# yzqin/s4g-release

Hardware: AMD Instinct MI355X
Metric: scenes/sec (25.6k-pt clouds) end-to-end grasp inference (higher is better)
Workload: dtype f32 (f16x2 split)

## Files before the change

s4g_release_amd/csrc/mlp_gemm.hip:

```cpp
#include <stdlib.h>

#include "mlp_common.h"

#include <type_traits>

#ifndef S4G_CHAIN_ABLATE
#define S4G_CHAIN_ABLATE 0
#endif

namespace s4g {


constexpr int GM_BM = 128;
constexpr int GM_BN = 128;
constexpr int GM_BK = 32;
constexpr int GM_LDS = 36;
constexpr int GM_THREADS = 256;

enum { LOAD_PLAIN = 0, LOAD_GATHER = 1, LOAD_INTERP = 2, LOAD_GATHER_MLP1 = 3, LOAD_GATHER_ADD = 4,
       LOAD_INTERP_ADD = 5, LOAD_CHANNEL_FIRST = 6,
       LOAD_REL_MLP1 = 64,
       LOAD_ADD_MFMA0 = 65 };
enum { EPI_STORE = 0, EPI_MAX = 1, EPI_CHANNEL_FIRST = 2, EPI_MAX_CF = 3 };

struct GemmParams {
  int P, Cin, Kpad, Cout, relu;
  const float* W;
  const float* bias;
  const float* A;
  int lda, a_coff, a_gcol;
  int aL;
  const int* gidx;
  const float* feat;
  const float* xyz;
  const float* ctr;
  int Cf, N, M, K;
  int nscenes;
  const float4* mlp1;
  const float4* rel4;
  const int* seg4;
  const int* seg_rows;
  float* out2;
  int ldc2, split_n;
  uint32_t* out_amax2;
  const int* nidx;
  const float* nw;
  const float* sparse;
  const float* dense;
  int C2, C1, N2, N1;
  float* out;
  int ldc, c_coff, c_gcol;
  int w_gstride, b_gstride;
  float* cf_ptr[4];
  int cf_start[5];
  int cf_sigmoid_from;
  int cf_N;
  int mtiles, ntiles;
  const uint16_t* W3;
  int Kpad16;
  int bf16_single;
  size_t w3_plane;
  const uint16_t* Wh2;
  const float* w_inv_scale;
  const float* a_amax;
  const float* a_amax2;
  float a_amax_floor;
  uint32_t* out_amax;
  int rps;
  const uint16_t* Wfrag;
  const float* lbias;
  const uint16_t* Wfrag2;
  const float* w_inv_scale2;
  const float* bias2;
  int Cout2, relu2;
  const uint16_t* Wfrag3;
  const float* w_inv_scale3;
  const float* bias3;
  int Cout3, relu3;
};

__device__ __forceinline__ float4 f4zero() { return make_float4(0.f, 0.f, 0.f, 0.f); }

__device__ __forceinline__ void gather_row_bm(int M, int K, int p0, int r, int& b, int& m) {
  const int MK = M * K;
  const int b0 = __builtin_amdgcn_readfirstlane(p0 / MK);
  int rem = p0 - b0 * MK + r;
  b = b0;
  while (rem >= MK) {
    rem -= MK;
    ++b;
  }
  m = (K & (K - 1)) == 0 ? rem >> (31 - __clz(K)) : rem / K;
}

template <int LOADER, int RPT = 4, int RS = 32>
struct ALoader {
  static __device__ __forceinline__ int srow(int t) { return LOADER == LOAD_CHANNEL_FIRST ? (t & 31) : (t >> 3); }
  static __device__ __forceinline__ int chunk(int t) { return LOADER == LOAD_CHANNEL_FIRST ? (t >> 5) : (t & 7); }
  const float* src0[RPT];
  bool ok[RPT];
  float rel[RPT][3];
  int i3[RPT][3];
  float w3[RPT][3];
  size_t drow[RPT];

  __device__ __forceinline__ void init(const GemmParams& p, int p0, int g, int t) {
    constexpr bool GATHERS = LOADER == LOAD_GATHER_MLP1 || LOADER == LOAD_GATHER_ADD || LOADER == LOAD_GATHER;
    int pp_[RPT], j_[RPT], b_[RPT], m_[RPT];
#pragma unroll
    for (int s = 0; s < RPT; ++s) {
      const int r = srow(t) + RS * s;
      const int pos = p0 + r;
      ok[s] = pos < p.P;
      pp_[s] = ok[s] ? pos : 0;
      j_[s] = b_[s] = m_[s] = 0;
      if constexpr (GATHERS) {
        if (!(LOADER == LOAD_GATHER_MLP1 && p.rel4)) {
          gather_row_bm(p.M, p.K, p0, ok[s] ? r : 0, b_[s], m_[s]);
          j_[s] = p.gidx[pp_[s]];
        }
      }
    }
#pragma unroll
    for (int s = 0; s < RPT; ++s) {
      const int pp = pp_[s], j = j_[s], b = b_[s], m = m_[s];
      if constexpr (LOADER == LOAD_PLAIN) {
        src0[s] = p.A + (size_t)pp * p.lda + p.a_coff + g * p.a_gcol;
      } else if constexpr (LOADER == LOAD_CHANNEL_FIRST) {
        const int b = pp / p.aL;
        src0[s] = p.A + (size_t)b * p.Cin * p.aL + (pp - b * p.aL);
      } else if constexpr (LOADER == LOAD_GATHER_MLP1) {
        if (p.rel4) {
          const float4 r4 = p.rel4[pp];
          rel[s][0] = r4.x;
          rel[s][1] = r4.y;
          rel[s][2] = r4.z;
          continue;
        }
        const float* x = p.xyz + (size_t)b * 3 * p.N;
        const float* c = p.ctr + (size_t)b * 3 * p.M;
        rel[s][0] = __fsub_rn(x[j], c[m]);
        rel[s][1] = __fsub_rn(x[p.N + j], c[p.M + m]);
        rel[s][2] = __fsub_rn(x[2 * p.N + j], c[2 * p.M + m]);
      } else if constexpr (LOADER == LOAD_GATHER_ADD) {
        src0[s] = p.feat + ((size_t)b * p.N + j) * p.Cf;
        const float* x = p.xyz + (size_t)b * 3 * p.N;
        const float* c = p.ctr + (size_t)b * 3 * p.M;
        rel[s][0] = __fsub_rn(x[j], c[m]);
        rel[s][1] = __fsub_rn(x[p.N + j], c[p.M + m]);
        rel[s][2] = __fsub_rn(x[2 * p.N + j], c[2 * p.M + m]);
      } else if constexpr (LOADER == LOAD_GATHER) {
        src0[s] = p.feat ? p.feat + ((size_t)b * p.N + j) * p.Cf : nullptr;
        if ((t & 7) == ((p.Cf & 31) >> 2)) {
          const float* x = p.xyz + (size_t)b * 3 * p.N;
          const float* c = p.ctr + (size_t)b * 3 * p.M;
          rel[s][0] = __fsub_rn(x[j], c[m]);
          rel[s][1] = __fsub_rn(x[p.N + j], c[p.M + m]);
          rel[s][2] = __fsub_rn(x[2 * p.N + j], c[2 * p.M + m]);
        }
      } else {
        const int bq = pp / p.N1;
#pragma unroll
        for (int k = 0; k < 3; ++k) {
          i3[s][k] = bq * p.N2 + p.nidx[(size_t)pp * 3 + k];
          w3[s][k] = p.nw[(size_t)pp * 3 + k];
        }
        drow[s] = (size_t)pp;
      }
    }
  }

  __device__ __forceinline__ float4 load(const GemmParams& p, int s, int k0, int t) const {
    if constexpr (LOADER == LOAD_GATHER_MLP1) {
      const bool live = ok[s] && k0 < p.Cin;
      const int kk = k0 < p.Cin ? k0 : 0;
      float4 r;
      float* rp = reinterpret_cast<float*>(&r);
#pragma unroll
      for (int e = 0; e < 4; ++e) {
        const float4 w = p.mlp1[kk + e];
        const float v = __fmaf_rn(w.z, rel[s][2], __fmaf_rn(w.y, rel[s][1], __fmaf_rn(w.x, rel[s][0], w.w)));
        rp[e] = live ? fmaxf(v, 0.f) : 0.f;
      }
      return r;
    }
    if constexpr (LOADER == LOAD_GATHER_ADD) {
      const bool live = ok[s] && k0 < p.Cin;
      const int kk = k0 < p.Cin ? k0 : 0;
      const float4 f = *reinterpret_cast<const float4*>(src0[s] + kk);
      const float fv[4] = {f.x, f.y, f.z, f.w};
      float4 r;
      float* rp = reinterpret_cast<float*>(&r);
#pragma unroll
      for (int e = 0; e < 4; ++e) {
        const float4 w = p.mlp1[kk + e];
        const float v = __fmaf_rn(w.z, rel[s][2], __fmaf_rn(w.y, rel[s][1], __fmaf_rn(w.x, rel[s][0], w.w)));
        rp[e] = live ? fmaxf(__fadd_rn(fv[e], v), 0.f) : 0.f;
// ... 986 lines not shown
    f32x16 z16;
#pragma unroll
    for (int r = 0; r < 16; ++r) z16[r] = 0.f;
#pragma unroll
    for (int rb = 0; rb < NRB; ++rb)
      asm volatile("s_nop 7" : "+v"(af0[rb][0].x), "+v"(af0[rb][0].y), "+v"(af0[rb][1].x), "+v"(af0[rb][1].y));
    __builtin_amdgcn_sched_barrier(0);
#pragma unroll
    for (int cb = 0; cb < 2; ++cb)
#pragma unroll
      for (int rb = 0; rb < NRB; ++rb) {
        acc[cb][rb] = chain_mfma<PL>(bf0[cb][1], af0[rb][0], z16);
        acc[cb][rb] = chain_mfma<PL>(bf0[cb][0], af0[rb][1], acc[cb][rb]);
        acc[cb][rb] = chain_mfma<PL>(bf0[cb][0], af0[rb][0], acc[cb][rb]);
      }
    if constexpr (ADD0) {
      float* Fs = smemf;
#pragma unroll
      for (int kt = 0; kt < NKT0; ++kt)
#pragma unroll
        for (int s = 0; s < RPT; ++s)
          *reinterpret_cast<float4*>(Fs + ((t >> 3) + RS * s) * fstr + kt * 32 + (t & 7) * 4) = fa[kt][s];
      __syncthreads();
#pragma unroll
      for (int nb = 0; nb < 2; ++nb)
#pragma unroll
        for (int j = 0; j < 4; ++j) {
          const float4 f4 = *reinterpret_cast<const float4*>(epi_s + nb * 32 + 8 * j + 4 * lh);
#pragma unroll
          for (int pb = 0; pb < NRB; ++pb) {
            const float4 fv = *reinterpret_cast<const float4*>(Fs + (wr * WROWS + pb * 32 + li) * fstr + wc * 64 + nb * 32 +
                                                               8 * j + 4 * lh);
            acc[nb][pb][4 * j] = __fmaf_rn(acc[nb][pb][4 * j], f4.x, fv.x);
            acc[nb][pb][4 * j + 1] = __fmaf_rn(acc[nb][pb][4 * j + 1], f4.y, fv.y);
            acc[nb][pb][4 * j + 2] = __fmaf_rn(acc[nb][pb][4 * j + 2], f4.z, fv.z);
            acc[nb][pb][4 * j + 3] = __fmaf_rn(acc[nb][pb][4 * j + 3], f4.w, fv.w);
          }
        }
      __syncthreads();
#pragma unroll
      for (int nb = 0; nb < 2; ++nb)
#pragma unroll
        for (int j = 0; j < 4; ++j)
#pragma unroll
          for (int pb = 0; pb < NRB; ++pb) {
            uint16_t* dst = Ah + (wr * WROWS + pb * 32 + li) * astr + wc * 64 + nb * 32 + 8 * j + 4 * lh;
            uint2 h, l;
            split_quad_h(fmaxf(acc[nb][pb][4 * j], 0.f), fmaxf(acc[nb][pb][4 * j + 1], 0.f),
                         fmaxf(acc[nb][pb][4 * j + 2], 0.f), fmaxf(acc[nb][pb][4 * j + 3], 0.f), sa, h.x, l.x, h.y, l.y);
            *reinterpret_cast<uint2*>(dst) = h;
            *reinterpret_cast<uint2*>(dst + aplane) = l;
          }
    } else {
#pragma unroll
      for (int nb = 0; nb < 2; ++nb)
#pragma unroll
        for (int j = 0; j < 4; ++j) {
          const float4 f4 = *reinterpret_cast<const float4*>(epi_s + nb * 32 + 8 * j + 4 * lh);
#pragma unroll
          for (int pb = 0; pb < NRB; ++pb) {
            uint16_t* dst = Ah + (wr * WROWS + pb * 32 + li) * astr + wc * 64 + nb * 32 + 8 * j + 4 * lh;
            uint2 h, l;
            split_quad_h2(fmaxf(acc[nb][pb][4 * j], 0.f), fmaxf(acc[nb][pb][4 * j + 1], 0.f),
                          fmaxf(acc[nb][pb][4 * j + 2], 0.f), fmaxf(acc[nb][pb][4 * j + 3], 0.f), f4.x, f4.y, f4.z, f4.w,
                          h.x, l.x, h.y, l.y);
            *reinterpret_cast<uint2*>(dst) = h;
            *reinterpret_cast<uint2*>(dst + aplane) = l;
          }
        }
    }
  } else {
    if (!(S4G_CHAIN_ABLATE & 16)) load_panel(0, std::integral_constant<int, (K / 32) / (NRB / 2)>{});
  }
  S4G_STAMP(2);
  __syncthreads();
  S4G_STAMP(3);

  auto zero_acc = [&]() {
#pragma unroll
    for (int i = 0; i < 2; ++i)
#pragma unroll
      for (int j = 0; j < NRB; ++j)
#pragma unroll
        for (int r = 0; r < 16; ++r) acc[i][j][r] = 0.f;
  };
  uint4 afn[NRB][PL];
  auto prime_a = [&]() {
#pragma unroll
    for (int rb = 0; rb < NRB; ++rb)
#pragma unroll
      for (int pl = 0; pl < PL; ++pl)
        afn[rb][pl] = *reinterpret_cast<const uint4*>(a_lane + pl * aplane + rb * 32 * astr);
  };

#define S4G_F2_STRIP(SWAPPED, ZFIRST, wcur, cbs_cur, wnext, cbs_next)                                                     \
  _Pragma("unroll") for (int ks = 0; ks < KS; ++ks) {                                                  \
    const int d = ks % GF_RING;                                                                        \
    const int ksn = ks + 1 == KS ? 0 : ks + 1;                                                         \
    uint4 af[NRB][PL], bf[2][PL];                                                                      \
    _Pragma("unroll") for (int rb = 0; rb < NRB; ++rb) _Pragma("unroll") for (int pl = 0; pl < PL; ++pl) { \
      af[rb][pl] = afn[rb][pl];                                                                        \
      if (!(S4G_CHAIN_ABLATE & 2))                                                                     \
        afn[rb][pl] = *reinterpret_cast<const uint4*>(a_lane + pl * aplane + rb * 32 * astr + ksn * 16); \
    }                                                                                                  \
    _Pragma("unroll") for (int cb = 0; cb < 2; ++cb) _Pragma("unroll") for (int pl = 0; pl < PL; ++pl)  \
      bf[cb][pl] = ring[d][cb][pl];                                                                    \
    {                                                                                                  \
      const int kr = ks + GF_RING;                                                                     \
      const WRef src = kr < KS ? (wcur) : (wnext);                                                     \
      const size_t cbs = kr < KS ? (cbs_cur) : (cbs_next);                                             \
      const int kk = kr < KS ? kr : kr - KS;                                                           \
      _Pragma("unroll") for (int cb = 0; cb < 2; ++cb) _Pragma("unroll") for (int pl = 0; pl < PL; ++pl) \
        if (!(S4G_CHAIN_ABLATE & 1))                                                                   \
          ring[d][cb][pl] = wref_load(src, wf_lane + pl * 1024, (uint32_t)(cb * cbs + (size_t)kk * PL * 1024)); \
    }                                                                                                  \
    if constexpr (PL == 2) {                                                                           \
      S4G_F2_TERM(SWAPPED, 0, 1, (ZFIRST) && ks == 0)                                                  \
      S4G_F2_TERM(SWAPPED, 1, 0, false)                                                                \
      S4G_F2_TERM(SWAPPED, 0, 0, false)                                                                \
    } else {                                                                                           \
      S4G_F2_TERM(SWAPPED, 0, 0, (ZFIRST) && ks == 0)                                                  \
    }                                                                                                  \
    _Pragma("unroll") for (int q = 0; q < 2 * PL; ++q) {                                               \
      __builtin_amdgcn_sched_group_barrier(0x008, 1, 0);                                               \
      __builtin_amdgcn_sched_group_barrier(0x100, 1, 0);                                               \
      __builtin_amdgcn_sched_group_barrier(0x008, 1, 0);                                               \
      __builtin_amdgcn_sched_group_barrier(0x020, 1, 0);                                               \
    }                                                                                                  \
    if constexpr (PL == 2) __builtin_amdgcn_sched_group_barrier(0x008, 4, 0);                          \
    if constexpr (PL == 1 && NRB == 4) {             \
      _Pragma("unroll") for (int q = 0; q < 2; ++q) {                                                  \
        __builtin_amdgcn_sched_group_barrier(0x100, 1, 0);                                             \
        __builtin_amdgcn_sched_group_barrier(0x008, 2, 0);                                             \
      }                                                                                                \
    }                                                                                                  \
    __builtin_amdgcn_sched_barrier(0);                                                                 \
  }
#define S4G_F2_TERM(SWAPPED, PA, PB, Z)                                                                \
  _Pragma("unroll") for (int cb = 0; cb < 2; ++cb) _Pragma("unroll") for (int rb = 0; rb < NRB; ++rb)  \
    if constexpr (SWAPPED)                                                                             \
      acc[cb][rb] = chain_mfma<PL>(bf[cb][PB], af[rb][PA], (Z) ? zero16 : acc[cb][rb]);                \
    else                                                                                               \
      acc[cb][rb] = chain_mfma<PL>(af[rb][PA], bf[cb][PB], (Z) ? zero16 : acc[cb][rb]);
  f32x16 zero16;
#pragma unroll
  for (int r = 0; r < 16; ++r) zero16[r] = 0.f;

  WRef wcur = w1;
  const float* __restrict__ scp = PL == 2 ? p.w_inv_scale + (size_t)g * p.b_gstride : nullptr;
  const float* __restrict__ bp = p.bias + (size_t)g * p.b_gstride;
  int relu_ph = p.relu;
  float inv_in = inv_sa, inv_sh = 1.f;
  const int npanel = tri ? 2 : 1;
  for (int ph = 0; ph < npanel; ++ph) {
  const WRef wnxt = ph + 1 < npanel ? wmid : (active0 ? w2 : wcur);
  prime_a();
  {
    const int n = wc * 64 + lane;
    epi_s[lane] = PL == 2 ? inv_in * scp[n] : 1.f;
    epi_s[64 + lane] = bp[n];
  }
  if (KC > 1 && ph == 0) {
    zero_acc();
    for (int kc = 0; kc < kchunks; ++kc) {
      if (kc > 0) {
        __syncthreads();
        load_panel(kc, std::integral_constant<int, 2>{});
        __syncthreads();
        prime_a();
      }
      const WRef wc1 = w1 + (size_t)kc * cb_stride;
      const bool lastc = kc + 1 == kchunks;
      const WRef wn1 = lastc ? wnxt : wc1 + cb_stride;
      const size_t cbsn = lastc ? cb_stride : cbs1;
      S4G_F2_STRIP(true, false, wc1, cbs1, wn1, cbsn)
    }
  } else {
    S4G_F2_STRIP(true, true, wcur, cb_stride, wnxt, cb_stride)
  }
  S4G_STAMP(4 + 4 * ph);
  if (S4G_CHAIN_ABLATE & 4) {
    chain_keep_alive(acc[0][0]); chain_keep_alive(acc[0][1]); chain_keep_alive(acc[1][0]); chain_keep_alive(acc[1][1]);
    __syncthreads();
    __syncthreads();
  } else {
  float tmax = 0.f;
  const float relu_lo = relu_ph ? 0.f : -__builtin_inff();
#pragma unroll
  for (int nb = 0; nb < 2; ++nb)
#pragma unroll
    for (int j = 0; j < 4; ++j) {
      const float4 sc4 = *reinterpret_cast<const float4*>(epi_s + nb * 32 + 8 * j + 4 * lh);
      const float4 b4 = *reinterpret_cast<const float4*>(epi_s + 64 + nb * 32 + 8 * j + 4 * lh);
      const float scv[4] = {sc4.x, sc4.y, sc4.z, sc4.w};
      const float bv[4] = {b4.x, b4.y, b4.z, b4.w};
#pragma unroll
      for (int pb = 0; pb < NRB; ++pb) {
        const f32x2 x01 = pk_fma(f32x2{acc[nb][pb][4 * j], acc[nb][pb][4 * j + 1]}, f32x2{scv[0], scv[1]}, f32x2{bv[0], bv[1]});
        const f32x2 x23 = pk_fma(f32x2{acc[nb][pb][4 * j + 2], acc[nb][pb][4 * j + 3]}, f32x2{scv[2], scv[3]}, f32x2{bv[2], bv[3]});
        const float x[4] = {fmaxf(x01.x, relu_lo), fmaxf(x01.y, relu_lo), fmaxf(x23.x, relu_lo), fmaxf(x23.y, relu_lo)};
#pragma unroll
        for (int e = 0; e < 4; ++e) acc[nb][pb][4 * j + e] = x[e];
        if constexpr (PL == 2) {
          tmax = fmaxf(fmaxf(tmax, fabsf(x[0])), fabsf(x[1]));
          tmax = fmaxf(fmaxf(tmax, fabsf(x[2])), fabsf(x[3]));
        }
      }
    }
  if constexpr (LOADER == LOAD_PLAIN && EPI2 == EPI_STORE) {
    if (!p.Wfrag2) {
      const bool second = p.split_n > 0 && g * p.c_gcol >= p.split_n;
      float* __restrict__ obase = second ? p.out2 - p.split_n : p.out + p.c_coff;
      const int old = second ? p.ldc2 : p.ldc;
      uint32_t* __restrict__ oamax = second ? p.out_amax2 : p.out_amax;
#pragma unroll
      for (int nb = 0; nb < 2; ++nb)
#pragma unroll
        for (int j = 0; j < 4; ++j) {
          const int nn = wc * 64 + nb * 32 + 8 * j + 4 * lh;
#pragma unroll
          for (int pb = 0; pb < NRB; ++pb) {
            const int row = p0 + wr * WROWS + pb * 32 + li;
            if (row < p.P)
              *reinterpret_cast<float4*>(obase + (size_t)row * old + g * p.c_gcol + nn) =
                  make_float4(acc[nb][pb][4 * j], acc[nb][pb][4 * j + 1], acc[nb][pb][4 * j + 2], acc[nb][pb][4 * j + 3]);
          }
        }
      if (PL == 2 && oamax) {
        const uint32_t wm = wave_max_u32(__float_as_uint(tmax));
        if (lane == 0) amax_publish(oamax, wm, (tile * 4 + wave) * 5 + g, p0, p_hi, p.rps);
      }
      return;
    }
  }
  float sh = 1.f;
  if constexpr (PL == 2) {
    const uint32_t wm = wave_max_u32(__float_as_uint(tmax));
    if (lane == 0) scr[NW * 128 + wave] = __uint_as_float(wm);
  }
  S4G_STAMP(5 + 4 * ph);
  __syncthreads();
  S4G_STAMP(6 + 4 * ph);
  if constexpr (PL == 2) {
    float hmax = scr[NW * 128];
#pragma unroll
    for (int w = 1; w < NW; ++w) hmax = fmaxf(hmax, scr[NW * 128 + w]);
    uint32_t exh = __float_as_uint(hmax) >> 23;
    exh = exh < 15u ? 15u : (exh > 240u ? 240u : exh);
    exh = __builtin_amdgcn_readfirstlane(exh);
    sh = __uint_as_float((268u - exh) << 23);
    inv_sh = __uint_as_float((exh - 14u) << 23);
  }
#pragma unroll
  for (int nb = 0; nb < 2; ++nb)
#pragma unroll
    for (int j = 0; j < 4; ++j)
#pragma unroll
      for (int pb = 0; pb < NRB; ++pb) {
        uint16_t* dst = Ah + (wr * WROWS + pb * 32 + li) * astr + wc * 64 + nb * 32 + 8 * j + 4 * lh;
        if constexpr (PL == 2) {
          const float4 v = make_float4(acc[nb][pb][4 * j], acc[nb][pb][4 * j + 1], acc[nb][pb][4 * j + 2],
                                       acc[nb][pb][4 * j + 3]);
          uint2 h, l;
          split2_h<false>(v, sh, h, l);
          *reinterpret_cast<uint2*>(dst) = h;
          *reinterpret_cast<uint2*>(dst + aplane) = l;
        } else {
          *reinterpret_cast<uint2*>(dst) = make_uint2(cvt_pk_bf16(acc[nb][pb][4 * j], acc[nb][pb][4 * j + 1]),
                                                      cvt_pk_bf16(acc[nb][pb][4 * j + 2], acc[nb][pb][4 * j + 3]));
        }
      }
  S4G_STAMP(7 + 4 * ph);
  __syncthreads();
  }
  inv_in = inv_sh;
  wcur = wmid;
  scp = PL == 2 ? p.w_inv_scale2 + (size_t)g * p.Cout2 : nullptr;
  bp = p.bias2 + (size_t)g * p.Cout2;
  relu_ph = p.relu2;
  }

  GemmParams q = p;
  q.Cout = CoutF;
  q.relu = tri ? p.relu3 : p.relu2;
  prime_a();
  WRef wstrip = w2;
  const float* __restrict__ bg2 = bgF;
  int sidv[NRB / 2][8] = {};
  if constexpr (SEGMAX) {
    if (seg_scene) {
#pragma unroll
      for (int c = 0; c < NRB / 2; ++c) {
        const int4* sp = reinterpret_cast<const int4*>(p.seg4 + ((p0 + wr * WROWS + c * 64 + lh * 32) >> 2));
        const int4 s0 = sp[0], s1 = sp[1];
        sidv[c][0] = s0.x; sidv[c][1] = s0.y; sidv[c][2] = s0.z; sidv[c][3] = s0.w;
        sidv[c][4] = s1.x; sidv[c][5] = s1.y; sidv[c][6] = s1.z; sidv[c][7] = s1.w;
      }
    }
  }
  for (int strip = 0; strip < nstrip2; ++strip, wstrip = wstrip + strip_stride) {
    if ((strip * CW + wc_u) * 64 >= CoutF) break;
    const int n = (strip * CW + wc) * 64 + lane;
    const float e_sc = PL == 2 ? inv_sh * scF[n] : 1.f;
    const float e_bias = bg2[n];
    const WRef wnext = ((strip + 1) * CW + wc_u) * 64 < CoutF ? wstrip + strip_stride : wstrip;
    S4G_STAMP(12 + 2 * (strip & 1));
    S4G_F2_STRIP(EPI2 == EPI_STORE, true, wstrip, cb_stride, wnext, cb_stride)
    S4G_STAMP(13 + 2 * (strip & 1));
    if (S4G_CHAIN_ABLATE & 8) {
      chain_keep_alive(acc[0][0]); chain_keep_alive(acc[0][1]); chain_keep_alive(acc[1][0]); chain_keep_alive(acc[1][1]);
      continue;
    }
    const int n0 = (strip * CW + wc) * 64;
    float omax = 0.f;
    if constexpr (EPI2 == EPI_STORE) {
      epi_s[lane] = e_sc;
      epi_s[64 + lane] = e_bias;
#pragma unroll
      for (int nb = 0; nb < 2; ++nb)
#pragma unroll
        for (int j = 0; j < 4; ++j) {
          const int nn = n0 + nb * 32 + 8 * j + 4 * lh;
          const float4 sc4 = *reinterpret_cast<const float4*>(epi_s + nb * 32 + 8 * j + 4 * lh);
          const float4 b4 = *reinterpret_cast<const float4*>(epi_s + 64 + nb * 32 + 8 * j + 4 * lh);
          const float scv[4] = {sc4.x, sc4.y, sc4.z, sc4.w};
          const float bv[4] = {b4.x, b4.y, b4.z, b4.w};
#pragma unroll
          for (int pb = 0; pb < NRB; ++pb) {
            float v[4];
#pragma unroll
            for (int e = 0; e < 4; ++e) {
              float x = __fmaf_rn(acc[nb][pb][4 * j + e], scv[e], bv[e]);
              if (q.relu) x = fmaxf(x, 0.f);
              v[e] = x;
              omax = fmaxf(omax, fabsf(x));
            }
            const int row = p0 + wr * WROWS + pb * 32 + li;
            if (row < p.P)
              *reinterpret_cast<float4*>(p.out + (size_t)row * p.ldc + p.c_coff + g * p.c_gcol + nn) =
                  make_float4(v[0], v[1], v[2], v[3]);
          }
        }
      if (p.out_amax) {
        const uint32_t wm = wave_max_u32(__float_as_uint(omax));
        if (lane == 0) amax_publish(p.out_amax, wm, tile * 4 + wave + strip, p0, p_hi, p.rps);
      }
    } else if (SEGMAX && seg_scene) {
      uint32_t* __restrict__ outu = reinterpret_cast<uint32_t*>(p.out);
#pragma unroll
      for (int cb = 0; cb < 2; ++cb) {
        const float sc = __shfl(e_sc, cb * 32 + li);
        const float bias = __shfl(e_bias, cb * 32 + li);
        const int nn = n0 + cb * 32 + li;
#pragma unroll
        for (int c = 0; c < NRB / 2; ++c) {
        float v[8];
#pragma unroll
        for (int qd = 0; qd < 4; ++qd) {
          const float o0 = fmaxf(fmaxf(acc[cb][2 * c][4 * qd], acc[cb][2 * c][4 * qd + 1]),
                                 fmaxf(acc[cb][2 * c][4 * qd + 2], acc[cb][2 * c][4 * qd + 3]));
          const float o1 = fmaxf(fmaxf(acc[cb][2 * c + 1][4 * qd], acc[cb][2 * c + 1][4 * qd + 1]),
                                 fmaxf(acc[cb][2 * c + 1][4 * qd + 2], acc[cb][2 * c + 1][4 * qd + 3]));
          const auto r = __builtin_amdgcn_permlane32_swap(__float_as_uint(o0), __float_as_uint(o1), false, false);
          v[2 * qd] = __uint_as_float(r[0]);
          v[2 * qd + 1] = __uint_as_float(r[1]);
        }
        auto emit = [&](int seg, float m) {
          if (seg < 0) return;
          const float x = fmaxf(m * sc + bias, 0.f);
          omax = fmaxf(omax, x);
          if (nn < CoutF) atomicMax(outu + (size_t)seg * p.ldc + p.c_coff + nn, __float_as_uint(x));
        };
        int cur = sidv[c][0];
        float m = v[0];
#pragma unroll
        for (int i = 1; i < 8; ++i) {
          const bool chg = sidv[c][i] != cur;
          if (chg) emit(cur, m);
          m = chg ? v[i] : fmaxf(m, v[i]);
          cur = sidv[c][i];
        }
        emit(cur, m);
        }
      }
      if (PL == 2 && p.out_amax) {
// ... 32 lines not shown
        const float bias = __shfl(e_bias, cb * 32 + li);
        float mx = -__builtin_inff(), mn = __builtin_inff();
#pragma unroll
        for (int rb = 0; rb < 2; ++rb)
#pragma unroll
          for (int r = 0; r < 16; ++r) {
            const float v = acc[cb][rb][r] * sc;
            acct[rb][cb][r] = v;
            mx = fmaxf(mx, v);
            mn = fminf(mn, v);
          }
        const float hi = mx + bias, lo = mn + bias;
        omax = fmaxf(omax, q.relu ? hi : fmaxf(fabsf(hi), fabsf(lo)));
      }
      if (p.out_amax) {
        const uint32_t wm = wave_max_u32(__float_as_uint(fmaxf(omax, 0.f)));
        if (lane == 0) amax_publish(p.out_amax, wm, tile * 4 + wave + strip, p0, p_hi, p.rps);
      }
      gemm_epilogue<EPI_MAX, 2>(q, acct, bg2, g, p0, n0, wave, wr, 0, li, lh, smemf);
    }
  }
  S4G_STAMP(11);
#undef S4G_F2_STRIP
#undef S4G_F2_TERM
}

template <int LOADER, int EPI2, int RW, int KC, int PL>
static int launch_mlp_chain(const GemmParams& p, int groups, hipStream_t st) {
  constexpr int CW = RW == 8 ? 8 : 4 / RW, RWN = RW == 8 ? 1 : RW;
  constexpr int NRB = PL == 1 ? S4G_CHAIN_BF16_NRB : 2;
  constexpr int BM = 32 * NRB * RWN, K = 64 * CW, NW = RWN * CW;
  constexpr size_t lds = sizeof(uint16_t) * PL * BM * (size_t)(K + 8) + sizeof(float) * (NW * 128 + 16);
  static_assert(lds <= (RW == 8 ? 160 : 80) * 1024, "two workgroups per CU (one for the 8-wave form)");
  static LdsAttrCache lds_cache;
  if (int rc = allow_dynamic_lds(reinterpret_cast<const void*>(&mlp_chain_kernel<LOADER, EPI2, RW, KC, PL>), lds, lds_cache)) return rc;
  const dim3 grid((unsigned)((p.P + BM - 1) / BM), (unsigned)groups);
  hipLaunchKernelGGL((mlp_chain_kernel<LOADER, EPI2, RW, KC, PL>), grid, dim3(64 * NW), lds, st, p);
  S4G_LAUNCH_CHECK();
  return S4G_OK;
}

template <int LOADER, int EPI, int PL = 2>
static int launch_gemm_f16x2(const GemmParams& p, int groups, hipStream_t st) {
  constexpr int force = 0;
  const int64_t wide_wgs = (int64_t)((p.P + GM_BM - 1) / GM_BM) * ((p.Cout + 255) / 256) * groups;
  const bool wide = force ? force == 4
                          : p.Cout > 256 && wide_wgs >= 512 &&
                                (LOADER == LOAD_PLAIN || LOADER == LOAD_GATHER_MLP1 || LOADER == LOAD_GATHER_ADD);
  if (wide) return launch_gemm_f16x2_cfg<LOADER, EPI, 4, PL>(p, groups, st);
  return launch_gemm_f16x2_cfg<LOADER, EPI, 2, PL>(p, groups, st);
}

template <int LOADER, int EPI, int NS, int WAVES>
static int launch_gemm_bf16x3_cfg(const GemmParams& p, int groups, hipStream_t st) {
  constexpr int BK = 32 * NS;
  size_t lds = sizeof(float) * GM_BM * (BK + 4) + sizeof(uint16_t) * 3 * GM_BN * (BK + 8);
  const size_t epi = sizeof(float) * 4 * 32 * 68;
  if (lds < epi) lds = epi;
  static LdsAttrCache lds_cache;
  if (int rc = allow_dynamic_lds(reinterpret_cast<const void*>(&mlp_gemm_bf16x3_kernel<LOADER, EPI, NS, WAVES>), lds, lds_cache)) return rc;
  const dim3 grid((unsigned)(p.mtiles * p.ntiles), (unsigned)groups);
  hipLaunchKernelGGL((mlp_gemm_bf16x3_kernel<LOADER, EPI, NS, WAVES>), grid, dim3(64 * WAVES), lds,
                     st, p);
  S4G_LAUNCH_CHECK();
  return S4G_OK;
}

template <int LOADER, int EPI>
static int launch_gemm_bf16x3(const GemmParams& p, int groups, hipStream_t st) {
  return launch_gemm_bf16x3_cfg<LOADER, EPI, 1, 4>(p, groups, st);
}

template <int LOADER, int EPI>
static int launch_gemm(const GemmParams& p, int groups, hipStream_t st) {
  const size_t lds = sizeof(float) * 2 * (GM_BM + GM_BN) * GM_LDS;
  static LdsAttrCache lds_cache;
  if (int rc = allow_dynamic_lds(reinterpret_cast<const void*>(&mlp_gemm_kernel<LOADER, EPI>), lds, lds_cache)) return rc;
  const dim3 grid((unsigned)(p.mtiles * p.ntiles), (unsigned)groups);
  hipLaunchKernelGGL((mlp_gemm_kernel<LOADER, EPI>), grid, dim3(GM_THREADS), lds, st, p);
  S4G_LAUNCH_CHECK();
  return S4G_OK;
}

}

#define S4G_FUSED2_LIST(X)                                                                       \
  X(LOAD_GATHER_MLP1, EPI_MAX, 2, 1)                                                             \
  X(LOAD_GATHER_MLP1, EPI_MAX, 1, 1)                                                             \
  X(LOAD_GATHER_ADD, EPI_MAX, 2, 1)                                                              \
  X(LOAD_GATHER_ADD, EPI_MAX, 1, 1)                                                              \
  X(LOAD_GATHER_ADD, EPI_MAX, 8, 1)       \
  X(LOAD_PLAIN, EPI_MAX, 2, 1)                                                                   \
  X(LOAD_PLAIN, EPI_MAX, 1, 1)                                                                   \
  X(LOAD_PLAIN, EPI_MAX, 8, 1)                                                                   \
  X(LOAD_PLAIN, EPI_STORE, 2, 1)                                                                 \
  X(LOAD_PLAIN, EPI_STORE, 1, 1)                                                                 \
  X(LOAD_PLAIN, EPI_STORE, 1, 2)            \
  X(LOAD_PLAIN, EPI_STORE, 1, 4)         \
  X(LOAD_PLAIN, EPI_STORE, 8, 1)                                                                 \
  X(LOAD_INTERP_ADD, EPI_STORE, 2, 1)                                                            \
  X(LOAD_INTERP_ADD, EPI_STORE, 1, 1)                                                            \
  X(LOAD_INTERP_ADD, EPI_STORE, 8, 1)

#ifdef S4G_CHAIN_STAMPS
extern "C" int s4g_debug_chain_stamps(unsigned long long* host_out_512x16) {
  return (int)hipMemcpyFromSymbol(host_out_512x16, HIP_SYMBOL(s4g::g_chain_stamps), sizeof(unsigned long long) * 512 * 16);
}
#endif

extern "C" int s4g_gemm_chain_supported(int loader, int epilogue, int C, int Kpad16) {
  using namespace s4g;
  const int r = C == 128 ? 2 : (C == 256 ? 1 : (C == 512 ? 8 : 0));
  if (r == 0 || Kpad16 <= 0 || Kpad16 % C) return 0;
  const int kc = Kpad16 / C;
#define S4G_FUSED2_Q(L, E, R, KCH) \
  if (loader == L && epilogue == (int)E && r == R && kc == KCH) return 1;
  S4G_FUSED2_LIST(S4G_FUSED2_Q)
#undef S4G_FUSED2_Q
  return 0;
}

extern "C" int s4g_mlp_gemm_f32(const s4g_gemm_desc_t* d, s4g_stream_t stream) {
  using namespace s4g;
  if (!d || d->P < 0 || d->Cout <= 0 || d->groups <= 0 || !d->bias) return S4G_EINVAL;
  const bool split = d->precision == S4G_GEMM_BF16X3 || d->precision == S4G_GEMM_BF16;
  const bool h2 = d->precision == S4G_GEMM_F16X2;
  if (h2) {
    if (!d->W_f16x2 || !d->w_inv_scale || d->Kpad16 <= 0 || (d->Kpad16 & 15) ||
        !(d->a_amax_floor >= 0.f) || (!d->a_amax && !d->a_amax2 && !(d->a_amax_floor > 0.f)))
      return S4G_EINVAL;
  } else if (split) {
    if (!d->W_bf16x3 || d->Kpad16 <= 0 || (d->Kpad16 & 15)) return S4G_EINVAL;
  } else if (d->precision == S4G_GEMM_FP32) {
    if (!d->W || d->Kpad <= 0 || (d->Kpad & 7)) return S4G_EINVAL;
  } else {
    return S4G_EINVAL;
  }
  if (d->P == 0) return S4G_OK;
  GemmParams p;
  p.P = d->P; p.Cin = d->Cin; p.Kpad = d->Kpad; p.Cout = d->Cout; p.relu = d->relu;
  p.W = d->W; p.bias = d->bias;
  p.A = d->A; p.lda = d->lda; p.a_coff = d->a_coff; p.a_gcol = d->a_gcol; p.aL = d->a_L;
  p.gidx = d->gidx; p.feat = d->feat; p.xyz = d->xyz; p.ctr = d->ctr;
  p.Cf = d->Cf; p.N = d->N; p.M = d->M; p.K = d->K;
  p.nscenes = d->M > 0 && d->K > 0 ? (int)((d->P + (int64_t)d->M * d->K - 1) / ((int64_t)d->M * d->K)) : 0;
  p.mlp1 = (const float4*)d->mlp1_w;
  p.rel4 = (const float4*)d->rel_xyz4;
  p.seg4 = d->seg4;
  p.seg_rows = d->seg_rows;
  p.out2 = d->out2;
  p.ldc2 = d->ldc2;
  p.split_n = d->out2 ? d->split_n : 0;
  p.out_amax2 = (uint32_t*)d->out_amax2;
  p.nidx = d->nidx; p.nw = d->nw; p.sparse = d->sparse; p.dense = d->dense;
  p.C2 = d->C2; p.C1 = d->C1; p.N2 = d->N2; p.N1 = d->N1;
  p.out = d->out; p.ldc = d->ldc; p.c_coff = d->c_coff; p.c_gcol = d->c_gcol;
  p.w_gstride = d->w_gstride; p.b_gstride = d->b_gstride;
  for (int i = 0; i < 4; ++i) p.cf_ptr[i] = d->cf_ptr[i];
  for (int i = 0; i < 5; ++i) p.cf_start[i] = d->cf_start[i];
  p.cf_sigmoid_from = d->cf_sigmoid_from; p.cf_N = d->cf_N;
  p.W3 = (const uint16_t*)d->W_bf16x3;
  p.Kpad16 = d->Kpad16;
  p.bf16_single = d->precision == S4G_GEMM_BF16 ? 1 : 0;
  p.w3_plane = (size_t)d->groups * (size_t)d->Cout * (size_t)d->Kpad16;
  p.Wh2 = (const uint16_t*)d->W_f16x2;
  p.w_inv_scale = d->w_inv_scale;
  p.a_amax = d->a_amax; p.a_amax2 = d->a_amax2; p.a_amax_floor = d->a_amax_floor;
  p.out_amax = (uint32_t*)d->out_amax;
  p.rps = d->rows_per_scene > 0 ? d->rows_per_scene : 0;
  p.Wfrag = (const uint16_t*)d->W_f16x2_frag;
  p.lbias = d->loader_bias;
  p.Wfrag2 = (const uint16_t*)d->W2_f16x2_frag;
  p.w_inv_scale2 = d->w2_inv_scale;
  p.bias2 = d->bias2;
  p.Cout2 = d->Cout2;
  p.relu2 = d->relu2;
  p.Wfrag3 = (const uint16_t*)d->W3_f16x2_frag;
  p.w_inv_scale3 = d->w3_inv_scale;
  p.bias3 = d->bias3;
  p.Cout3 = d->Cout3;
  p.relu3 = d->relu3;
  p.mtiles = (d->P + GM_BM - 1) / GM_BM;
  p.ntiles = (d->Cout + GM_BN - 1) / GM_BN;
  hipStream_t st = (hipStream_t)stream;

  if (d->loader == S4G_GEMM_LOAD_PLAIN) {
    if (!d->A || (d->lda & 3) || (d->a_coff & 3) || (d->a_gcol & 3) || (d->Cin & 3)) return S4G_EINVAL;
  } else if (d->loader == S4G_GEMM_LOAD_GATHER) {
    if (!d->gidx || !d->xyz || !d->ctr || (d->Cf & 3) || (d->Cf > 0 && !d->feat) ||
        d->K <= 0 || d->M <= 0 || d->N <= 0 || d->groups != 1)
      return S4G_EINVAL;
  } else if (d->loader == S4G_GEMM_LOAD_GATHER_MLP1) {
    if ((!d->rel_xyz4 && (!d->gidx || !d->xyz || !d->ctr)) || ((uintptr_t)d->rel_xyz4 & 15) ||
        !d->mlp1_w || (d->Cin & 3) || d->K <= 0 || d->M <= 0 || d->N <= 0 || d->groups != 1 ||
        ((uintptr_t)d->mlp1_w & 15))
      return S4G_EINVAL;
    if ((d->seg4 != nullptr) != (d->seg_rows != nullptr)) return S4G_EINVAL;
    if (d->seg4 && (!d->rel_xyz4 || !d->W2_f16x2_frag || d->epilogue != S4G_GEMM_EPI_MAX || d->K != 64 ||
                    d->rows_per_scene <= 0 || (d->rows_per_scene & 255) || !d->relu2 || d->W3_f16x2_frag))
      return S4G_EINVAL;
  } else if (d->loader == S4G_GEMM_LOAD_GATHER_ADD) {
    if (!d->gidx || !d->xyz || !d->ctr || !d->mlp1_w || !d->feat || (d->Cin & 3) || d->Cf != d->Cin ||
        d->K <= 0 || d->M <= 0 || d->N <= 0 || d->groups != 1 || ((uintptr_t)d->mlp1_w & 15) ||
        ((uintptr_t)d->feat & 15))
      return S4G_EINVAL;
  } else if (d->loader == S4G_GEMM_LOAD_INTERP_ADD) {
    if (!d->nidx || !d->nw || !d->sparse || !d->loader_bias || (d->Cin & 3) || d->C2 != d->Cin ||
        d->N1 <= 0 || d->N2 <= 0 || d->groups != 1 ||
        (((uintptr_t)d->sparse | (uintptr_t)d->dense | (uintptr_t)d->loader_bias) & 15))
      return S4G_EINVAL;
  } else if (d->loader == S4G_GEMM_LOAD_INTERP) {
    if (!d->nidx || !d->nw || !d->sparse || (d->C2 & 3) || (d->C1 & 3) ||
        (d->C1 > 0 && !d->dense) || d->N1 <= 0 || d->N2 <= 0 || d->groups != 1)
      return S4G_EINVAL;
  } else if (d->loader == S4G_GEMM_LOAD_CHANNEL_FIRST) {
    if (!d->A || d->Cin < 1 || d->a_L <= 0 || d->P % d->a_L || d->groups != 1 ||
        d->Cin > (h2 ? d->Kpad16 : d->Kpad))
      return S4G_EINVAL;
  } else {
    return S4G_EINVAL;
  }
  if (d->loader != S4G_GEMM_LOAD_GATHER_MLP1 && (d->seg4 || d->seg_rows)) return S4G_EINVAL;
  if (d->out2) {
    const bool bf1_ = d->precision == S4G_GEMM_BF16;
    if (!(h2 || bf1_) || d->loader != S4G_GEMM_LOAD_PLAIN || d->epilogue != S4G_GEMM_EPI_STORE || d->W2_f16x2_frag ||
        d->groups != 1 || d->split_n <= 0 || (d->split_n & 255) || d->split_n >= d->Cout || (d->Cout & 255) ||
        (d->ldc2 & 3) || ((uintptr_t)d->out2 & 15) || d->c_coff != 0 || (d->ldc & 3) || ((uintptr_t)d->out & 15))
      return S4G_EINVAL;
  }
  if (d->epilogue == S4G_GEMM_EPI_MAX) {
    if (!(d->K == 16 || d->K == 32 || d->K == 64) || d->groups != 1 || !d->out) return S4G_EINVAL;
  } else if (d->epilogue == S4G_GEMM_EPI_STORE) {
    if (!d->out) return S4G_EINVAL;
  } else if (d->epilogue == S4G_GEMM_EPI_CHANNEL_FIRST) {
    if (d->cf_N <= 0 || d->groups != 1) return S4G_EINVAL;
  } else if (d->epilogue == S4G_GEMM_EPI_MAX_CHANNEL_FIRST) {
    if (d->relu != 1 || d->K < 1 || d->M < 1 || d->P % ((int64_t)d->M * d->K) || d->groups != 1 || !d->out ||
        d->W2_f16x2_frag || d->out2)
      return S4G_EINVAL;
  } else {
    return S4G_EINVAL;
  }

  if (d->W2_f16x2_frag) {
    const bool c128 = d->Cout == 128 && d->Kpad16 == 128,
               c256 = d->Cout == 256 && (d->Kpad16 == 256 || d->Kpad16 == 512),
               c512 = d->Cout == 512 && d->Kpad16 == 512;
    const bool store = d->epilogue == S4G_GEMM_EPI_STORE;
    const bool bf1 = d->precision == S4G_GEMM_BF16;
    if ((!h2 && !bf1) || (!store && (d->epilogue != S4G_GEMM_EPI_MAX || d->K != 64 || (d->P & 63))) ||
        (!c128 && !c256 && !c512) || d->Cout2 <= 0 || (d->Cout2 & 63) || (!store && d->groups != 1) || !d->W_f16x2_frag ||
        (d->W3_f16x2_frag && (d->Cout2 != d->Cout || d->Cout3 <= 0 || (d->Cout3 & 63) ||
                              (h2 && !d->w3_inv_scale) || !d->bias3)) ||
        (h2 && !d->w2_inv_scale) || !d->bias2 ||
        (store && (((d->ldc | d->c_coff | d->c_gcol) & 3) || ((uintptr_t)d->out & 15))))
      return S4G_EINVAL;
    if (h2 && d->loader == S4G_GEMM_LOAD_GATHER_MLP1 && d->rel_xyz4 && d->epilogue == S4G_GEMM_EPI_MAX &&
        d->Kpad16 == d->Cout && d->Cin <= d->Cout && (c128 || c256)) {
      const char* m0 = s4g::knob("S4G_MLP1_MFMA");
      if (!(m0 && m0[0] == '0'))
        return c128 ? launch_mlp_chain<LOAD_REL_MLP1, EPI_MAX, 2, 1, 2>(p, d->groups, st)
                    : launch_mlp_chain<LOAD_REL_MLP1, EPI_MAX, 1, 1, 2>(p, d->groups, st);
    }
    if (h2 && d->loader == S4G_GEMM_LOAD_GATHER_ADD && d->epilogue == S4G_GEMM_EPI_MAX && d->Kpad16 == d->Cout &&
        (int64_t)p.nscenes * d->N * d->Cf * 4 < (1ll << 31) && (int64_t)p.nscenes * d->N * 12 < (1ll << 31))
      return c128   ? launch_mlp_chain<LOAD_ADD_MFMA0, EPI_MAX, 2, 1, 2>(p, d->groups, st)
             : c256 ? launch_mlp_chain<LOAD_ADD_MFMA0, EPI_MAX, 1, 1, 2>(p, d->groups, st)
                    : launch_mlp_chain<LOAD_ADD_MFMA0, EPI_MAX, 8, 1, 2>(p, d->groups, st);
#define S4G_FUSED2_CASE(L, E, R, KCH)                                                        \
  if (d->loader == L && (int)d->epilogue == (int)E && (c128 ? 2 : (c256 ? 1 : 8)) == R &&     \
      d->Kpad16 / d->Cout == KCH)                                                             \
    return bf1 ? launch_mlp_chain<L, E, R, KCH, 1>(p, d->groups, st)                 \
               : launch_mlp_chain<L, E, R, KCH, 2>(p, d->groups, st);
    S4G_FUSED2_LIST(S4G_FUSED2_CASE)
#undef S4G_FUSED2_CASE
    return S4G_EUNSUPPORTED;
  }
  {
    const char* sc_env = s4g::knob("S4G_GEMM_SINGLE_CHAIN");
    const bool single_chain = !(sc_env && sc_env[0] == '0');
    const bool bf1 = d->precision == S4G_GEMM_BF16;
    const int kc = d->Kpad16 / 256;
    if (single_chain && (h2 || bf1) && d->loader == S4G_GEMM_LOAD_PLAIN && d->epilogue == S4G_GEMM_EPI_STORE &&
        d->W_f16x2_frag && d->groups == 1 && d->Cout % 256 == 0 && d->Kpad16 % 256 == 0 &&
        (kc == 1 || kc == 2 || kc == 4) && ((d->ldc | d->c_coff) & 3) == 0 && ((uintptr_t)d->out & 15) == 0 &&
        (d->Cout >= 1024 || d->Kpad16 >= 1024 || (sc_env && sc_env[0] == '1'))) {
      GemmParams q = p;
      q.Cout = 256;
      q.a_gcol = 0;
      q.c_gcol = 256;
      q.b_gstride = 256;
      const int strips = d->Cout / 256;
#define S4G_SINGLE_CASE(KCH)                                                                     \
  if (kc == KCH)                                                                                 \
    return bf1 ? launch_mlp_chain<LOAD_PLAIN, EPI_STORE, 1, KCH, 1>(q, strips, st)               \
               : launch_mlp_chain<LOAD_PLAIN, EPI_STORE, 1, KCH, 2>(q, strips, st);
      S4G_SINGLE_CASE(1)
      S4G_SINGLE_CASE(2)
      S4G_SINGLE_CASE(4)
#undef S4G_SINGLE_CASE
    }
  }
  constexpr bool bf16_tiled = true;
#define S4G_GEMM_CASE(L, E)                                            \
  if (d->loader == L && d->epilogue == E)                              \
    return h2 ? launch_gemm_f16x2<L, E>(p, d->groups, st)              \
           : (p.bf16_single && bf16_tiled) ? launch_gemm_f16x2<L, E, 1>(p, d->groups, st) \
           : split ? launch_gemm_bf16x3<L, E>(p, d->groups, st)        \
                   : launch_gemm<L, E>(p, d->groups, st);
  S4G_GEMM_CASE(LOAD_PLAIN, EPI_STORE)
  S4G_GEMM_CASE(LOAD_PLAIN, EPI_MAX)
  S4G_GEMM_CASE(LOAD_PLAIN, EPI_CHANNEL_FIRST)
  S4G_GEMM_CASE(LOAD_GATHER, EPI_STORE)
  S4G_GEMM_CASE(LOAD_GATHER, EPI_MAX)
  S4G_GEMM_CASE(LOAD_INTERP, EPI_STORE)
  S4G_GEMM_CASE(LOAD_GATHER_MLP1, EPI_STORE)
  S4G_GEMM_CASE(LOAD_GATHER_MLP1, EPI_MAX)
  S4G_GEMM_CASE(LOAD_GATHER_ADD, EPI_STORE)
  S4G_GEMM_CASE(LOAD_GATHER_ADD, EPI_MAX)
  S4G_GEMM_CASE(LOAD_INTERP_ADD, EPI_STORE)
#undef S4G_GEMM_CASE
#define S4G_GEMM_CASE_CF(L, E)                                                           \
  if (d->loader == L && d->epilogue == E)                                                \
    return h2 ? launch_gemm_f16x2<L, E>(p, d->groups, st)                                \
              : d->precision == S4G_GEMM_FP32 ? launch_gemm<L, E>(p, d->groups, st) : S4G_EUNSUPPORTED;
  S4G_GEMM_CASE_CF(LOAD_CHANNEL_FIRST, EPI_STORE)
  S4G_GEMM_CASE_CF(LOAD_CHANNEL_FIRST, EPI_CHANNEL_FIRST)
  S4G_GEMM_CASE_CF(LOAD_CHANNEL_FIRST, EPI_MAX_CF)
  S4G_GEMM_CASE_CF(LOAD_PLAIN, EPI_MAX_CF)
#undef S4G_GEMM_CASE_CF
  return S4G_EUNSUPPORTED;
}

__global__ __launch_bounds__(256) void amax_per_scene_kernel(const float* __restrict__ x, int64_t n,
                                                             uint32_t* __restrict__ slots) {
  const int b = blockIdx.y;
  const float* xs = x + (size_t)b * n;
  float m = 0.f;
  for (int64_t i = (int64_t)blockIdx.x * 256 + threadIdx.x; i < n; i += (int64_t)gridDim.x * 256)
    m = fmaxf(m, fabsf(xs[i]));
  const uint32_t wm = s4g::wave_max_u32(__float_as_uint(m));
  if ((threadIdx.x & 63) == 0) atomicMax(slots + (size_t)b * 64 + ((blockIdx.x * 4 + (threadIdx.x >> 6)) & 63), wm);
}

extern "C" int s4g_amax_per_scene_f32(const float* x, int64_t B, int64_t n_per_scene, float* out_slots,
                                      s4g_stream_t stream) {
  if (B < 0 || n_per_scene < 0 || B > 65535 || ((!x || !out_slots) && B * n_per_scene > 0)) return S4G_EINVAL;
  if (B == 0 || n_per_scene == 0) return S4G_OK;
  const int64_t want = (n_per_scene + 256 * 16 - 1) / (256 * 16);
  const unsigned wgs = (unsigned)(want < 64 ? want : 64);
  hipLaunchKernelGGL(amax_per_scene_kernel, dim3(wgs, (unsigned)B), dim3(256), 0, (hipStream_t)stream, x, n_per_scene,
                     reinterpret_cast<uint32_t*>(out_slots));
  S4G_LAUNCH_CHECK();
  return S4G_OK;
}
```

Measured before the change: 2063.

## Loop over output strips inside single-chain kernel to reuse A panel for K=256

For single-chunk (K=256) plain-store GEMMs with large P, the launch now uses one group and has each block iterate over all 256-wide output strips in-kernel. The A panel stays resident while weights, bias and scales advance per strip. The single-chain path is also enabled for Cout>=768 in this case. This removes repeated A-panel loads and extra block launches, but gives fewer blocks, each running longer and serialising the strips.

```diff
diff --git a/s4g_release_amd/csrc/mlp_gemm.hip b/s4g_release_amd/csrc/mlp_gemm.hip
--- a/s4g_release_amd/csrc/mlp_gemm.hip
+++ b/s4g_release_amd/csrc/mlp_gemm.hip
@@ -43,6 +43,7 @@
   float* out2;
   int ldc2, split_n;
   uint32_t* out_amax2;
+  int nstrip1;
   const int* nidx;
   const float* nw;
   const float* sparse;
@@ -1335,8 +1336,11 @@
   int relu_ph = p.relu;
   float inv_in = inv_sa, inv_sh = 1.f;
   const int npanel = tri ? 2 : 1;
+  constexpr bool SL_STRIPS = LOADER == LOAD_PLAIN && EPI2 == EPI_STORE && KC == 1;
+  int sl_strip = 0;
   for (int ph = 0; ph < npanel; ++ph) {
-  const WRef wnxt = ph + 1 < npanel ? wmid : (active0 ? w2 : wcur);
+  const bool sl_more = SL_STRIPS && sl_strip + 1 < p.nstrip1;
+  const WRef wnxt = sl_more ? wcur + strip_stride : (ph + 1 < npanel ? wmid : (active0 ? w2 : wcur));
   prime_a();
   {
     const int n = wc * 64 + lane;
@@ -1392,7 +1396,8 @@
     }
   if constexpr (LOADER == LOAD_PLAIN && EPI2 == EPI_STORE) {
     if (!p.Wfrag2) {
-      const bool second = p.split_n > 0 && g * p.c_gcol >= p.split_n;
+      const int sl_col = sl_strip * K;
+      const bool second = p.split_n > 0 && g * p.c_gcol + sl_col >= p.split_n;
       float* __restrict__ obase = second ? p.out2 - p.split_n : p.out + p.c_coff;
       const int old = second ? p.ldc2 : p.ldc;
       uint32_t* __restrict__ oamax = second ? p.out_amax2 : p.out_amax;
@@ -1400,7 +1405,7 @@
       for (int nb = 0; nb < 2; ++nb)
 #pragma unroll
         for (int j = 0; j < 4; ++j) {
-          const int nn = wc * 64 + nb * 32 + 8 * j + 4 * lh;
+          const int nn = sl_col + wc * 64 + nb * 32 + 8 * j + 4 * lh;
 #pragma unroll
           for (int pb = 0; pb < NRB; ++pb) {
             const int row = p0 + wr * WROWS + pb * 32 + li;
@@ -1411,9 +1416,15 @@
         }
       if (PL == 2 && oamax) {
         const uint32_t wm = wave_max_u32(__float_as_uint(tmax));
-        if (lane == 0) amax_publish(oamax, wm, (tile * 4 + wave) * 5 + g, p0, p_hi, p.rps);
-      }
-      return;
+        if (lane == 0) amax_publish(oamax, wm, (tile * 4 + wave) * 5 + g + sl_strip, p0, p_hi, p.rps);
+      }
+      if (!sl_more) return;
+      ++sl_strip;
+      wcur = wcur + strip_stride;
+      if constexpr (PL == 2) scp += K;
+      bp += K;
+      --ph;
+      continue;
     }
   }
   float sh = 1.f;
@@ -1752,6 +1763,7 @@
   p.ldc2 = d->ldc2;
   p.split_n = d->out2 ? d->split_n : 0;
   p.out_amax2 = (uint32_t*)d->out_amax2;
+  p.nstrip1 = 1;
   p.nidx = d->nidx; p.nw = d->nw; p.sparse = d->sparse; p.dense = d->dense;
   p.C2 = d->C2; p.C1 = d->C1; p.N2 = d->N2; p.N1 = d->N1;
   p.out = d->out; p.ldc = d->ldc; p.c_coff = d->c_coff; p.c_gcol = d->c_gcol;
@@ -1884,13 +1896,18 @@
     if (single_chain && (h2 || bf1) && d->loader == S4G_GEMM_LOAD_PLAIN && d->epilogue == S4G_GEMM_EPI_STORE &&
         d->W_f16x2_frag && d->groups == 1 && d->Cout % 256 == 0 && d->Kpad16 % 256 == 0 &&
         (kc == 1 || kc == 2 || kc == 4) && ((d->ldc | d->c_coff) & 3) == 0 && ((uintptr_t)d->out & 15) == 0 &&
-        (d->Cout >= 1024 || d->Kpad16 >= 1024 || (sc_env && sc_env[0] == '1'))) {
+        (d->Cout >= 1024 || d->Kpad16 >= 1024 || (kc == 1 && d->Cout >= 768 && d->P >= 64 * 512) ||
+         (sc_env && sc_env[0] == '1'))) {
       GemmParams q = p;
       q.Cout = 256;
       q.a_gcol = 0;
       q.c_gcol = 256;
       q.b_gstride = 256;
-      const int strips = d->Cout / 256;
+      int strips = d->Cout / 256;
+      if (kc == 1 && strips > 1 && d->P >= 64 * 512) {
+        q.nstrip1 = strips;
+        strips = 1;
+      }
 #define S4G_SINGLE_CASE(KCH)                                                                     \
   if (kc == KCH)                                                                                 \
     return bf1 ? launch_mlp_chain<LOAD_PLAIN, EPI_STORE, 1, KCH, 1>(q, strips, st)               \
```

After: 2068, median of 6. Within noise of the previous version (+0.2%).
